# rpng/R-VIO

Measured on AMD Instinct MI355X. Metric: camera frames/sec (KLT+RANSAC track, IMU propagate, MSCKF update, augment/compose), 200 feat / 10-clone window, higher is better.
Workload: dtype f64 (filter) / u8+i32+f32 (KLT); 1 GPU; cfgB: synthetic EuRoC-shaped 752x480 @20Hz, 200 features, 10-clone window, IMU 200 Hz, single stream, equalizer on (CLAHE 3.0, 5x5), corners from the device detector (GFTT + cornerSubPix); parallelism=single GPU

## Files before the change

r-vio_amd/abi.py:

```python
import ctypes as C
import math
import numpy as np

ABI_VERSION = 6

RVIO_PIX_MONO8, RVIO_PIX_RGB8, RVIO_PIX_BGR8, RVIO_PIX_RGBA8, RVIO_PIX_BGRA8 = 0, 1, 2, 3, 4
PIX_CHANNELS = {RVIO_PIX_MONO8: 1, RVIO_PIX_RGB8: 3, RVIO_PIX_BGR8: 3, RVIO_PIX_RGBA8: 4, RVIO_PIX_BGRA8: 4}


class rvio_config(C.Structure):
    _fields_ = [
        ("imu_rate", C.c_double), ("sigma_g", C.c_double), ("sigma_wg", C.c_double),
        ("sigma_a", C.c_double), ("sigma_wa", C.c_double), ("gravity", C.c_double),
        ("small_angle", C.c_double),
        ("width", C.c_int32), ("height", C.c_int32),
        ("fx", C.c_float), ("fy", C.c_float), ("cx", C.c_float), ("cy", C.c_float),
        ("k1", C.c_float), ("k2", C.c_float), ("p1", C.c_float), ("p2", C.c_float), ("k3", C.c_float),
        ("sigma_px", C.c_float), ("sigma_py", C.c_float),
        ("T_bc", C.c_double * 16),
        ("fisheye", C.c_int32),
        ("n_features", C.c_int32), ("max_track_len", C.c_int32), ("min_track_len", C.c_int32),
        ("min_dist", C.c_float), ("qual_lvl", C.c_float),
        ("block_x", C.c_float), ("block_y", C.c_float),
        ("enable_equalizer", C.c_int32), ("use_sampson", C.c_int32),
        ("inlier_thr", C.c_double),
        ("ini_thr_angle", C.c_double), ("ini_thr_displ", C.c_double),
        ("ini_enable_alignment", C.c_int32), ("reserved0", C.c_int32),
    ]


class rvio_imu(C.Structure):
    _fields_ = [("w", C.c_double * 3), ("a", C.c_double * 3), ("t", C.c_double), ("dt", C.c_double)]


IMU_DTYPE = np.dtype([("w", "f8", 3), ("a", "f8", 3), ("t", "f8"), ("dt", "f8")])
assert IMU_DTYPE.itemsize == C.sizeof(rvio_imu) == 64


class rvio_tracks(C.Structure):
    _fields_ = [("n_feat", C.c_int32), ("max_len", C.c_int32),
# ... 188 lines not shown
```

r-vio_amd/csrc/detector.hip:

```cpp
#pragma once

#define DET_NBCAP 64
#define DET_FAST_N 2048
#define DET_FAST_CELLS 4096

struct DetDev {
    const int* first;
    float* eig;
    int* maxkey;
    int* counters;
    int* cell_cnt;
    unsigned long long* cell_ent;
    int* cell_ci;
    int* nb;
    int* nb_cnt;
    int n_cap;
    unsigned long long* prov;
    unsigned long long* cand;
    unsigned long long* acc;
    unsigned char* state;
    float* raw_xy;
    float* xy;
    int* n_out;
    const float* spmask;
    int sp_win;
    int W, H, F;
    float min_dist;
    double quality;
    int max_cells;
};

__device__ __forceinline__ void det_shift(DetDev& d, size_t off) {
    zmove(d.first, off); zmove(d.eig, off); zmove(d.maxkey, off); zmove(d.counters, off); zmove(d.cell_cnt, off); zmove(d.cell_ent, off);
    zmove(d.cell_ci, off); zmove(d.nb, off); zmove(d.nb_cnt, off); zmove(d.prov, off); zmove(d.cand, off); zmove(d.acc, off); zmove(d.state, off);
    zmove(d.raw_xy, off); zmove(d.xy, off); zmove(d.n_out, off);
}
// ... 326 lines not shown
    if (n_list > 0) flush();
}

__device__ __forceinline__ void det_geometry(const DetDev& d, float* md, int* cell, int* gw, int* gh) {
    const float s = (*d.first) ? 1.f : 2.f;
    *md = s * d.min_dist;
    *cell = (int)rintf(*md);
    *gw = (d.W + *cell - 1) / *cell; *gh = (d.H + *cell - 1) / *cell;
}

#define NMS_T 256
__global__ __launch_bounds__(NMS_T) void nms_threshold_kernel(DetDev d, size_t bs) {
    det_shift(d, (size_t)blockIdx.z * bs);
    const int W = d.W;
    const int np = d.counters[3];
    const float mx = ord2f(*d.maxkey);
    const float thr = (float)((double)mx * d.quality);
    float md; int cell, gw, gh;
    det_geometry(d, &md, &cell, &gw, &gh);
    for (int i = blockIdx.x * NMS_T + threadIdx.x; i < np; i += gridDim.x * NMS_T) {
        const unsigned long long key = d.prov[i];
        const float v = __int_as_float((int)(key >> 32));
        if (!(v > thr)) continue;
        const int idx = (int)(key & 0xffffffffull), x = idx % W, y = idx / W;
        const int ci = atomicAdd(&d.counters[0], 1);
        d.cand[ci] = key;
        const int c = (y / cell) * gw + (x / cell);
        const size_t slot = (size_t)c * cell * cell + atomicAdd(&d.cell_cnt[c], 1);
        d.cell_ent[slot] = key;
        d.cell_ci[slot] = ci;
    }
}

#define NEIGH_T 1024
#define NEIGH_BLOCKS 8
#define NEIGH_BLOCKS_WIDE 2
#define NEIGH_LDS (DET_FAST_N * (8 + 4 + 2 + 2 + 2) + (DET_FAST_CELLS + 2) * 4)

__global__ __launch_bounds__(NEIGH_T) void neigh_kernel(DetDev d, size_t bs) {
    det_shift(d, (size_t)blockIdx.z * bs);
    extern __shared__ __align__(16) unsigned char ndyn[];
    __shared__ int s_w[16];
    const int W = d.W, tid = threadIdx.x;
    float md; int cell, gw, gh;
    det_geometry(d, &md, &cell, &gw, &gh);
    const double md2 = (double)md * (double)md;
    const int n = d.counters[0], ncell = gw * gh;
    if (n <= DET_FAST_N && ncell <= DET_FAST_CELLS) {
        unsigned long long* fkey = (unsigned long long*)ndyn;
        unsigned int* fxy = (unsigned int*)(fkey + DET_FAST_N);
        int* cstart = (int*)(fxy + DET_FAST_N);
        unsigned short* fcell = (unsigned short*)(cstart + DET_FAST_CELLS + 2);
        unsigned short* fslot = fcell + DET_FAST_N;
        unsigned short* order = fslot + DET_FAST_N;
        for (int c = tid; c < ncell; c += NEIGH_T) cstart[c] = 0;
        __syncthreads();
        for (int c = tid; c < n; c += NEIGH_T) {
            const unsigned long long key = d.cand[c];
            const int idx = (int)(key & 0xffffffffull), x = idx % W, y = idx / W;
            const int cc = (y / cell) * gw + (x / cell);
            fkey[c] = key; fxy[c] = (unsigned)x | ((unsigned)y << 16); fcell[c] = (unsigned short)cc;
            fslot[c] = (unsigned short)atomicAdd(&cstart[cc], 1);
        }
        __syncthreads();
        {
            const int per = (ncell + NEIGH_T - 1) / NEIGH_T, b0 = tid * per, lane = tid & 63, wv = tid >> 6;
            int sum = 0;
            for (int k = 0; k < per; ++k) if (b0 + k < ncell) sum += cstart[b0 + k];
            const int inc = wave_incl_scan(sum);
            if (lane == 63) s_w[wv] = inc;
            __syncthreads();
            int run = inc - sum;
            for (int w = 0; w < wv; ++w) run += s_w[w];
            for (int k = 0; k < per; ++k) if (b0 + k < ncell) { const int c = cstart[b0 + k]; cstart[b0 + k] = run; run += c; }
            if (tid == NEIGH_T - 1) cstart[ncell] = run;
        }
        __syncthreads();
        for (int c = tid; c < n; c += NEIGH_T) order[cstart[fcell[c]] + fslot[c]] = (unsigned short)c;
        __syncthreads();
        for (int c = blockIdx.x * NEIGH_T + tid; c < n; c += gridDim.x * NEIGH_T) {
            const unsigned long long key = fkey[c];
            const int x = (int)(fxy[c] & 0xffffu), y = (int)(fxy[c] >> 16), xc = x / cell, yc = y / cell;
            const int y1 = yc > 0 ? yc - 1 : 0, y2 = yc + 1 < gh ? yc + 1 : gh - 1, x1 = xc > 0 ? xc - 1 : 0, x2 = xc + 1 < gw ? xc + 1 : gw - 1;
            int m = 0;
            int* list = d.nb + (size_t)c * DET_NBCAP;
            for (int yy = y1; yy <= y2; ++yy) {
                const int e0 = cstart[yy * gw + x1], e1 = cstart[yy * gw + x2 + 1];
                for (int e = e0; e < e1; ++e) {
                    const int j = order[e];
                    if (!(fkey[j] > key)) continue;
                    const float ddx = (float)x - (float)(fxy[j] & 0xffffu), ddy = (float)y - (float)(fxy[j] >> 16);
                    if ((double)(ddx * ddx + ddy * ddy) < md2) { if (m < DET_NBCAP) list[m] = j; ++m; }
                }
            }
            d.nb_cnt[c] = m <= DET_NBCAP ? m : -1;
        }
        return;
    }
    const size_t cap = (size_t)cell * cell;
    for (int c = blockIdx.x * NEIGH_T + tid; c < n && c < d.n_cap; c += gridDim.x * NEIGH_T) {
        const unsigned long long key = d.cand[c];
        const int idx = (int)(key & 0xffffffffull);
        const int x = idx % W, y = idx / W, xc = x / cell, yc = y / cell;
        int cnt9[9], cid9[9];
#pragma unroll
        for (int q = 0; q < 9; ++q) {
            const int xx = xc + (q % 3) - 1, yy = yc + (q / 3) - 1;
            const bool in = xx >= 0 && yy >= 0 && xx < gw && yy < gh;
            cid9[q] = in ? yy * gw + xx : 0;
            cnt9[q] = in ? d.cell_cnt[cid9[q]] : 0;
        }
        int m = 0;
        int* list = d.nb + (size_t)c * DET_NBCAP;
#pragma unroll
        for (int q = 0; q < 9; ++q) {
            const unsigned long long* ent = d.cell_ent + (size_t)cid9[q] * cap;
            const int* eci = d.cell_ci + (size_t)cid9[q] * cap;
            for (int e = 0; e < cnt9[q]; ++e) {
                const unsigned long long k2 = ent[e];
                if (!(k2 > key)) continue;
                const int i2 = (int)(k2 & 0xffffffffull);
                const float ddx = (float)x - (float)(i2 % W), ddy = (float)y - (float)(i2 / W);
                if ((double)(ddx * ddx + ddy * ddy) < md2) { if (m < DET_NBCAP) list[m] = eci[e]; ++m; }
            }
        }
        d.nb_cnt[c] = m <= DET_NBCAP ? m : -1;
    }
}

#define GREEDY_T 1024
#define DET_LDS_ST 32768
__device__ __noinline__ int greedy_general_step(const DetDev& d, int c, int m, unsigned char* lst, int cell, int gw, int gh, double md2) {
    volatile unsigned char* ls = lst;
    volatile unsigned char* gs = d.state;
    const int W = d.W;
    bool drop = false, wait = false;
    auto st_get = [&](int ci) -> unsigned char { return ci < DET_LDS_ST ? ls[ci] : gs[ci]; };
    if (m >= 0) {
        const int* list = d.nb + (size_t)c * DET_NBCAP;
        for (int e = 0; e < m; ++e) { const unsigned char s2 = st_get(list[e]); drop |= (s2 == 2); wait |= (s2 == 1); }
    } else {
        const size_t cap = (size_t)cell * cell;
        const unsigned long long key = d.cand[c];
        const int idx = (int)(key & 0xffffffffull);
        const int x = idx % W, y = idx / W, xc = x / cell, yc = y / cell;
        const int x1 = xc > 0 ? xc - 1 : 0, y1 = yc > 0 ? yc - 1 : 0, x2 = xc + 1 < gw ? xc + 1 : gw - 1, y2 = yc + 1 < gh ? yc + 1 : gh - 1;
        for (int yy = y1; yy <= y2; ++yy)
            for (int xx = x1; xx <= x2; ++xx) {
                const int cc = yy * gw + xx, cnt = d.cell_cnt[cc];
                const unsigned long long* ent = d.cell_ent + (size_t)cc * cap;
                const int* eci = d.cell_ci + (size_t)cc * cap;
                for (int e = 0; e < cnt; ++e) {
                    const unsigned long long k2 = ent[e];
                    if (!(k2 > key)) continue;
                    const int i2 = (int)(k2 & 0xffffffffull);
                    const float ddx = (float)x - (float)(i2 % W), ddy = (float)y - (float)(i2 / W);
                    if ((double)(ddx * ddx + ddy * ddy) < md2) { const unsigned char s2 = st_get(eci[e]); drop |= (s2 == 2); wait |= (s2 == 1); }
                }
            }
    }
    return (drop ? 1 : 0) | (wait ? 2 : 0);
}
#define DET_LDS_TK 4096
#define DET_CL_N 2048
#define DET_CL_CAP 24576
#define GREEDY_LDS (DET_LDS_TK * 8 + DET_LDS_ST + DET_CL_CAP * 2 + (DET_CL_N + 4) * 4)
__global__ __launch_bounds__(GREEDY_T) void greedy_kernel(DetDev d, size_t bs) {
    det_shift(d, (size_t)blockIdx.z * bs);
    extern __shared__ __align__(16) unsigned char gdyn[];
    unsigned long long* tk = (unsigned long long*)gdyn;
    unsigned char* lst = gdyn + DET_LDS_TK * 8;
    unsigned short* clist = (unsigned short*)(lst + DET_LDS_ST);
    int* coff = (int*)(clist + DET_CL_CAP);
    __shared__ int s_w[16];
    __shared__ int s_flag;
    const int W = d.W, tid = threadIdx.x;
    float md; int cell, gw, gh;
    det_geometry(d, &md, &cell, &gw, &gh);
    const double md2 = (double)md * (double)md;
    const int n = d.counters[0];
    volatile unsigned char* ls = lst;
    volatile unsigned char* gs = d.state;
#define ST_GET(ci) ((ci) < DET_LDS_ST ? ls[(ci)] : gs[(ci)])
#define ST_SET(ci, v) do { if ((ci) < DET_LDS_ST) ls[(ci)] = (v); else gs[(ci)] = (v); } while (0)
    DBG_T(56);
    for (int c = tid; c < n; c += GREEDY_T) ST_SET(c, 1);
    bool packed = n <= DET_CL_N && n <= d.n_cap;
    if (tid == 0) s_flag = 0;
    __syncthreads();
    if (packed) {
        const int c0 = 2 * tid, c1 = 2 * tid + 1, lane = tid & 63, wv = tid >> 6;
        const int m0 = c0 < n ? d.nb_cnt[c0] : 0, m1 = c1 < n ? d.nb_cnt[c1] : 0;
        if (m0 < 0 || m1 < 0) s_flag = 1;
        const int sum = (m0 > 0 ? m0 : 0) + (m1 > 0 ? m1 : 0);
        const int inc = wave_incl_scan(sum);
        if (lane == 63) s_w[wv] = inc;
        __syncthreads();
        int base = inc - sum;
        for (int w = 0; w < wv; ++w) base += s_w[w];
        if (tid == GREEDY_T - 1 && base + sum > DET_CL_CAP) s_flag = 1;
        __syncthreads();
        packed = (s_flag == 0);
        if (packed) {
            auto copy_list = [&](int c, int dst, int m) {
                const int4* l4 = (const int4*)(d.nb + (size_t)c * DET_NBCAP);
                for (int q = 0; q < m; q += 16) {
                    const int4 v0 = l4[q / 4], v1 = l4[q / 4 + 1], v2 = l4[q / 4 + 2], v3 = l4[q / 4 + 3];
                    const int v[16] = {v0.x, v0.y, v0.z, v0.w, v1.x, v1.y, v1.z, v1.w, v2.x, v2.y, v2.z, v2.w, v3.x, v3.y, v3.z, v3.w};
#pragma unroll
                    for (int u = 0; u < 16; ++u) if (q + u < m) clist[dst + q + u] = (unsigned short)v[u];
                }
            };
            if (c0 < n) { coff[c0] = base; copy_list(c0, base, m0); }
            if (c1 < n) { coff[c1] = base + m0; copy_list(c1, base + m0, m1); }
            if (c0 == n - 1) coff[n] = base + m0;
            if (c1 == n - 1) coff[n] = base + m0 + m1;
        }
    }
    __threadfence_block();
    __syncthreads();
    DBG_T(57);
    int pending, rounds = 0;
    do {
        pending = 0; ++rounds;
        if (rounds == 1) DBG_T(10);
        for (int c = tid; c < n; c += GREEDY_T) {
            if (ST_GET(c) != 1) continue;
            bool drop = false, wait = false;
            const int m = packed ? -2 : (c < d.n_cap ? d.nb_cnt[c] : -1);
            if (m == -2) {
                const int o = coff[c], o1 = coff[c + 1];
                for (int e = o; e < o1 && !drop; e += 8) {
                    int id8[8];
#pragma unroll
                    for (int u = 0; u < 8; ++u) id8[u] = (int)clist[min(e + u, o1 - 1)];
                    unsigned char s8[8];
#pragma unroll
                    for (int u = 0; u < 8; ++u) s8[u] = lst[id8[u]];
#pragma unroll
                    for (int u = 0; u < 8; ++u) { drop |= (s8[u] == 2); wait |= (s8[u] == 1); }
                }
            } else {
                const int dw = greedy_general_step(d, c, m, lst, cell, gw, gh, md2);
                drop = (dw & 1) != 0; wait = (dw & 2) != 0;
            }
            if (rounds == 1) DBG_T(11);
            if (drop) ST_SET(c, 3);
            else if (!wait) ST_SET(c, 2);
            else pending = 1;
        }
        if (rounds == 1) DBG_T(12);
        __threadfence_block();
        pending = __syncthreads_or(pending);
        if (rounds == 1) DBG_T(13);
        if (rounds == 2) DBG_T(14);
    } while (pending);
    DBG_T(59);
#ifdef RVIO_DBG_CLOCKS
    if (tid == 0) { g_dbg[62] = n; g_dbg[63] = rounds; }
#endif
    if (tid == 0) s_flag = 0;
    __syncthreads();
    const bool small = n <= DET_LDS_TK;
    for (int c = tid; c < n; c += GREEDY_T)
        if (ST_GET(c) == 2) {
            const unsigned long long key = d.cand[c];
            if (small) tk[atomicAdd(&s_flag, 1)] = key;
            else d.acc[atomicAdd(&d.counters[1], 1)] = key;
        }
#undef ST_GET
#undef ST_SET
    __threadfence_block();
    __syncthreads();
    const int na = small ? s_flag : ((volatile int*)d.counters)[1];
    const bool in_lds = small || na <= DET_LDS_TK;
    if (!small && in_lds) for (int a = tid; a < na; a += GREEDY_T) tk[a] = d.acc[a];
    __syncthreads();
    for (int a = tid; a < na; a += GREEDY_T) {
        const unsigned long long key = in_lds ? tk[a] : d.acc[a];
        int r = 0;
        if (in_lds) for (int b = 0; b < na; ++b) r += (tk[b] > key) ? 1 : 0;
        else for (int b = 0; b < na; ++b) r += (d.acc[b] > key) ? 1 : 0;
        if (r < d.F) {
            const int idx = (int)(key & 0xffffffffull);
            d.raw_xy[2 * r] = (float)(idx % W); d.raw_xy[2 * r + 1] = (float)(idx / W);
        }
    }
    DBG_T(60);
    if (tid == 0) {
        *d.n_out = na < d.F ? na : d.F;
        *d.maxkey = (int)0x80000000;
        d.counters[3] = 0;
    }
}

#define SP_WIN 7
#define SP_WW (2 * SP_WIN + 1)
#define SP_PW (SP_WW + 2)
#define SP_MARG 12
#define SP_RS (SP_PW + 1 + 2 * SP_MARG)
#define SP_T 256
#define SP_LS 44
__global__ __launch_bounds__(SP_T) void subpix_kernel(const uint8_t* __restrict__ src, int stride, DetDev d, size_t src_bs, size_t bs, int dbg_tag) {
    DBG_I(blockIdx.x == 0 && blockIdx.z == 0, dbg_tag, 2);
    src = zoff(src, src_bs); det_shift(d, (size_t)blockIdx.z * bs);
    __shared__ unsigned char reg[SP_RS * SP_RS];
    __shared__ double s_part[2][4][5];
    const int p = blockIdx.x, tid = threadIdx.x, lane = tid & 63, wv = tid >> 6;
    const int n = *d.n_out;
    if (p >= n) return;
    const int W = d.W, H = d.H;
    const float tx = d.raw_xy[2 * p], ty = d.raw_xy[2 * p + 1];
    const int rx0 = (int)tx - (SP_PW - 1) / 2 - SP_MARG, ry0 = (int)ty - (SP_PW - 1) / 2 - SP_MARG;
    for (int e = tid; e < SP_RS * SP_RS; e += SP_T) {
        const int j = e / SP_RS, i = e % SP_RS;
        reg[e] = src[(size_t)min(max(ry0 + j, 0), H - 1) * stride + min(max(rx0 + i, 0), W - 1)];
    }
    __syncthreads();
    auto pix = [&](int x, int y) -> float {
        const int i = x - rx0, j = y - ry0;
        if ((unsigned)i < (unsigned)SP_RS && (unsigned)j < (unsigned)SP_RS) return (float)reg[j * SP_RS + i];
// ... 402 lines not shown
```

r-vio_amd/csrc/rvio_hip.hip:

```cpp
#include <hip/hip_runtime.h>
#include <atomic>
#include <chrono>
#include <dlfcn.h>
#include <cmath>
#include <cstdio>
#include <cstdlib>
#include <cstring>
#include <map>
#include <mutex>
#include <string>
#include <vector>

#include "../../include/rvio_hip.h"
#include "rvio_dev.h"
#include "frontend_dev.h"
#include "filter_kernels.hip"
#include "filter_kernels2.hip"
#include "solve6.hip"
#include "solve7.hip"
#include "solve9.hip"
#include "landmarks.hip"
#include "odom.hip"
#pragma clang fp contract(off)
#include "frontend_kernels.hip"
// ... 1102 lines not shown
    const DevCfg& d = h->dc;
    int rc = RVIO_OK;
    for (int k = 0; k < h->plan.n_ic; ++k) if ((rc = detector_alloc_set(h, h->dets[k])) != RVIO_OK) return rc;
    for (int k = h->plan.n_ic; k < rvio_hip::kIC; ++k) h->dets[k] = h->dets[0];
    DALLOC(h, h->det_xy2[0], (size_t)2 * d.F); DALLOC(h, h->det_xy2[1], (size_t)2 * d.F); DALLOC(h, h->det_xy2[2], (size_t)2 * d.F);
    DALLOC(h, h->det_nout, 3);
    float* mask = nullptr;
    const size_t mside = (size_t)std::max(31, 2 * (int)std::floor(.5 * h->cfg.min_dist) + 1);
    DALLOC(h, mask, mside * mside);
    for (DetDev* q : {&h->dets[0], &h->dets[1], &h->dets[2]}) { q->xy = h->det_xy2[0]; q->n_out = h->det_nout; q->spmask = mask; q->sp_win = (int)std::floor(.5 * h->cfg.min_dist); }
    return RVIO_OK;
}
static int detector_init(rvio_hip* h) {
    if (h->det_ready) return RVIO_OK;
    int rc = detector_check(h);
    if (rc != RVIO_OK) return rc;
    if (!h->det_in_slab && (rc = detector_alloc(h)) != RVIO_OK) return rc;
    DetDev& q = h->dets[0];
    const int spw = q.sp_win, spww = 2 * spw + 1;
    std::vector<float> hm((size_t)spww * spww);
    for (int i = 0; i < spww; ++i) {
        const float y = (float)(i - spw) / (float)spw;
        const float vy = std::exp(-y * y);
        for (int j = 0; j < spww; ++j) { const float x = (float)(j - spw) / (float)spw; hm[(size_t)i * spww + j] = (float)(vy * std::exp(-x * x)); }
    }
    HIPCHK(h, hipMemcpyAsync(const_cast<float*>(q.spmask), hm.data(), sizeof(float) * hm.size(), hipMemcpyHostToDevice, h->stream));
    HIPCHK(h, hipStreamSynchronize(h->stream));
    if (spw > 15) HIPCHK(h, lds_attr((const void*)subpix_wide_kernel, (int)subpix_wide_lds(spw)));
    std::vector<int> minkey((size_t)h->batch, (int)0x80000000);
    for (DetDev* qq : {&h->dets[0], &h->dets[1], &h->dets[2]})
        HIPCHK(h, hipMemcpy2DAsync(qq->maxkey, h->slab_bytes ? h->slab_bytes : sizeof(int), minkey.data(), sizeof(int), sizeof(int), (size_t)(h->det_in_slab ? h->batch : 1),
                                   hipMemcpyHostToDevice, h->stream));
    HIPCHK(h, hipStreamSynchronize(h->stream));
    HIPCHK(h, lds_attr((const void*)neigh_kernel, (int)NEIGH_LDS));
    HIPCHK(h, lds_attr((const void*)greedy_kernel, (int)GREEDY_LDS));
    h->det_ready = true;
    return RVIO_OK;
}
static DetDev det_view(const rvio_hip* h) {
    DetDev q = h->dets[h->runahead ? h->ic : 0];
    q.xy = h->det_xy2[h->dslot]; q.n_out = h->det_nout + h->dslot;
    return q;
}
static hipStream_t image_stream_of(const rvio_hip* h, int ic) { return ic == 0 ? h->stream_t : h->stream_c; }
static hipStream_t image_stream(const rvio_hip* h) { return h->runahead ? image_stream_of(h, h->ic) : h->ts; }
static int detect_dev(rvio_hip* h, const uint8_t* img, int stride, size_t src_bs, hipEvent_t first_flag_ready) {
    const DevCfg& d = h->dc;
    const size_t bs = h->slab_bytes;
    const unsigned B = (unsigned)h->batch;
    const DetDev q = det_view(h);
    const hipStream_t ds = image_stream(h);
    h->det_set_last = h->runahead ? h->ic : 0;
    if (h->wide_px) {
        if (h->pyr_signal) { hipLaunchKernelGGL(stage_signal_kernel, dim3(1), dim3(64), 0, ds, h->pyr_signal); h->pyr_signal = nullptr; }
        hipLaunchKernelGGL(mineig_nms_strip_kernel, dim3((d.W + DET_SW - 1) / DET_SW, (d.H + DET_SH - 1) / DET_SH, B), dim3(64), 0, ds, img, stride, q, src_bs, bs);
    } else {
        hipLaunchKernelGGL(mineig_nms_kernel, dim3((d.W + DET_TW - 1) / DET_TW, (d.H + DET_FH - 1) / DET_FH, B), dim3(DET_T), 0, ds, img, stride, q, src_bs, bs, (int)h->frame_no, h->pyr_signal);
        h->pyr_signal = nullptr;
    }
    if (first_flag_ready) HIPCHK(h, hipStreamWaitEvent(ds, first_flag_ready, 0));
    hipLaunchKernelGGL(nms_threshold_kernel, dim3(16, 1, B), dim3(NMS_T), 0, ds, q, bs);
    const unsigned neigh_blocks = h->wide_px ? NEIGH_BLOCKS_WIDE : NEIGH_BLOCKS;
    hipLaunchKernelGGL(neigh_kernel, dim3(neigh_blocks, 1, B), dim3(NEIGH_T), NEIGH_LDS, ds, q, bs);
    hipLaunchKernelGGL(greedy_kernel, dim3(1, 1, B), dim3(GREEDY_T), GREEDY_LDS, ds, q, bs);
    launch_subpix(h, q, img, stride, src_bs, B, (int)h->frame_no, ds);
    HIPCHK(h, hipGetLastError());
    return RVIO_OK;
}

static int pix_channels(int fmt) { return fmt == RVIO_PIX_MONO8 ? 1 : (fmt == RVIO_PIX_RGB8 || fmt == RVIO_PIX_BGR8) ? 3 : 4; }
static void launch_gray(rvio_hip* h, const uint8_t* src, int stride, size_t src_bs, uint8_t* dst, hipStream_t st) {
    const DevCfg& d = h->dc;
    const int bgr = (h->pix_fmt == RVIO_PIX_BGR8 || h->pix_fmt == RVIO_PIX_BGRA8) ? 1 : 0;
    const size_t bs = (size_t)d.W * d.H;
    const dim3 g((d.W + 255) / 256, (d.H + 3) / 4, h->batch), b(256);
    const bool wide = d.W % 4 == 0 && stride % 4 == 0 && ((uintptr_t)src & 3) == 0 && src_bs % 4 == 0;
    if (h->pix_ch == 3) {
        if (wide) hipLaunchKernelGGL(gray_kernel4<3>, g, b, 0, st, src, d.W, d.H, stride, bgr, dst, src_bs, bs);
        else hipLaunchKernelGGL(gray_kernel<3>, g, b, 0, st, src, d.W, d.H, stride, bgr, dst, src_bs, bs);
    } else {
        if (wide) hipLaunchKernelGGL(gray_kernel4<4>, g, b, 0, st, src, d.W, d.H, stride, bgr, dst, src_bs, bs);
        else hipLaunchKernelGGL(gray_kernel<4>, g, b, 0, st, src, d.W, d.H, stride, bgr, dst, src_bs, bs);
    }
}
int rvio_hip_get_image_format(const rvio_hip* h) { return h ? h->pix_fmt : RVIO_ERR_INVALID; }
int rvio_hip_set_image_format(rvio_hip* h, int format) {
    if (!h) return RVIO_ERR_INVALID;
    if (format < RVIO_PIX_MONO8 || format > RVIO_PIX_BGRA8) { h->err = "unknown image format"; return RVIO_ERR_INVALID; }
    if (format != RVIO_PIX_MONO8 && !h->front_end) { h->err = "this batch handle was created without its front end: it takes no image"; return RVIO_ERR_UNSUPPORTED; }
    if (format == h->pix_fmt) return RVIO_OK;
    HIPCHK(h, hipSetDevice(h->device));
    { const int rc = drain_all(h); if (rc != RVIO_OK) return rc; }
    const int ch = pix_channels(format);
    const size_t npx = (size_t)h->dc.W * h->dc.H;
    if (ch > 1 && !h->d_gray[0]) {
        uint8_t* p = nullptr;
        HIPCHK(h, hipMalloc((void**)&p, 4 * npx * (size_t)h->batch));
// ... 532 lines not shown
        HIPCHK(h, hipMemcpyAsync(h->hb_img[b], pp, npx, hipMemcpyHostToDevice, h->stream_t));
        if (nc > 0) HIPCHK(h, hipMemcpyAsync(h->hb_cand[b], pp + pin_cand, sizeof(float) * 2 * nc, hipMemcpyHostToDevice, h->stream_t));
        HIPCHK(h, hipEventRecord(h->evPin[ps], h->stream_t));
    }
    h->last_ra = ra;
    if (paranoid_bits() & PAR_SYNC_COPIES) {
        HIPCHK(h, hipStreamSynchronize(h->stream_d));
        HIPCHK(h, hipStreamSynchronize(h->stream_t));
        if (h->stream_c) HIPCHK(h, hipStreamSynchronize(h->stream_c));
    }
    return frame_dev_impl(h, h->hb_img[b], (int)rowb, h->hb_imu[imu_slot], m, cand_xy ? h->hb_cand[b] : nullptr, nc, true);
}
int rvio_hip_frame_points(rvio_hip* h, const float* tracked_xy, const unsigned char* status, int n_pts,
                          const rvio_imu* imu, int m, const float* cand_xy, int n_cand) {
    int rc = rvio_hip_track_points(h, tracked_xy, status, n_pts, imu, m, cand_xy, n_cand);
    if (rc != RVIO_OK) return rc;
    return frame_tail_dev(h, h->d_imu, m);
}

int rvio_hip_get_frame_info(rvio_hip* h, rvio_frame_info* info) {
    if (!h || !info) return RVIO_ERR_INVALID;
    HIPCHK(h, hipSetDevice(h->device));
    SYNC_FRONT(h);
    FilterMeta m;
    double lit_rank = -1.0;
    HIPCHK(h, hipMemcpyAsync(info, h->d_info, sizeof *info, hipMemcpyDeviceToHost, h->stream));
    HIPCHK(h, hipMemcpyAsync(&m, h->meta, sizeof m, hipMemcpyDeviceToHost, h->stream));
    if (h->last_Ab) HIPCHK(h, hipMemcpyAsync(&lit_rank, h->last_Ab + (size_t)h->dc.ldh * (h->dc.ldh - 1) + 5, sizeof lit_rank, hipMemcpyDeviceToHost, h->stream));
    HIPCHK(h, hipStreamSynchronize(h->stream));
    info->n_clones = h->n_clones_host; info->n_feat_accepted = m.n_good; info->n_rows = m.n_rows; info->updated = m.updated;
    info->reserved[0] = m.err;
    info->reserved[1] = (m.updated && lit_rank >= 0) ? (int)lit_rank : -1;
    info->rank_truncated_at = m.updated ? m.trunc_at : -1;
    if (m.err & 4) { h->err = "a device-side stage counter timed out (filter -> book-keeping): the frame sequence is invalid, re-initialise"; return RVIO_ERR_STATE; }
    return RVIO_OK;
}
int rvio_hip_get_pose(rvio_hip* h, double p[3], double q[4]) {
    if (!h) return RVIO_ERR_INVALID;
    HIPCHK(h, hipSetDevice(h->device));
    double buf[8];
    HIPCHK(h, hipMemcpyAsync(buf, h->d_pose, sizeof buf, hipMemcpyDeviceToHost, h->stream));
    HIPCHK(h, hipStreamSynchronize(h->stream));
    if (p) for (int i = 0; i < 3; ++i) p[i] = buf[i];
    if (q) for (int i = 0; i < 4; ++i) q[i] = buf[3 + i];
    return RVIO_OK;
}
int rvio_hip_get_pose_at(rvio_hip* h, int instance, double p[3], double q[4]) {
    if (!h || instance < 0 || instance >= h->batch) return RVIO_ERR_INVALID;
    HIPCHK(h, hipSetDevice(h->device));
    double buf[8];
    HIPCHK(h, hipMemcpyAsync(buf, (const char*)h->d_pose + (size_t)instance * h->slab_bytes, sizeof buf, hipMemcpyDeviceToHost, h->stream));
    HIPCHK(h, hipStreamSynchronize(h->stream));
    if (p) for (int i = 0; i < 3; ++i) p[i] = buf[i];
    if (q) for (int i = 0; i < 4; ++i) q[i] = buf[3 + i];
    return RVIO_OK;
}

}

extern "C" {
int rvio_hip_get_corners(rvio_hip* h, int32_t* n, float* xy, float* raw_xy, float* eig) {
    if (!h) return RVIO_ERR_INVALID;
    FRONT_END_ONLY(h);
    if (!h->det_ready) { h->err = "the device detector has not run (pass a NULL corner list to track/frame)"; return RVIO_ERR_INVALID; }
    HIPCHK(h, hipSetDevice(h->device));
    SYNC_FRONT(h);
// ... 62 lines not shown
        if (h->batch > 1 || !h->plan.fuse_ok || !h->time_imu || n < 1) return RVIO_ERR_UNSUPPORTED;
        HIPCHK(h, hipMalloc(&bx, sizeof(double) * d.xdmax)); HIPCHK(h, hipMalloc(&bP, sizeof(double) * d.dmax * d.dmax));
        HIPCHK(h, hipMemcpyAsync(bx, h->x[h->cur], sizeof(double) * d.xdmax, hipMemcpyDeviceToDevice, h->stream));
        HIPCHK(h, hipMemcpyAsync(bP, h->P[h->cur], sizeof(double) * d.dmax * d.dmax, hipMemcpyDeviceToDevice, h->stream));
    }
    if (which == 11 && (h->pix_ch < 2 || !h->gray_src)) { h->err = "no colour image has been handed over (rvio_hip_set_image_format)"; return RVIO_ERR_UNSUPPORTED; }
    rvio_odom* odt = nullptr;
    if (which == 12) {
        if (!h->odom_ring) { h->err = "the odometry ring was never enabled (rvio_hip_set_odometry)"; return RVIO_ERR_UNSUPPORTED; }
        HIPCHK(h, hipMalloc((void**)&odt, sizeof(rvio_odom) * h->batch));
    }
    LmOut lmt = {nullptr, nullptr, nullptr, nullptr, 0};
    if (which == 10) {
        if (!h->lm.count) return RVIO_ERR_UNSUPPORTED;
        const int rc = lm_alloc(h, &lmt);
        if (rc != RVIO_OK) return rc;
    }
    const bool pre = h->plan.solve9_nt && (h->plan.solve9_nt <= 6 || h->plan.chol_queue);
    const UpdateForms fw = forms_at(h, n, pre, true), fs = forms_at(h, n, pre, false);
    HIPCHK(h, hipEventCreate(&e0)); HIPCHK(h, hipEventCreate(&e1));
    HIPCHK(h, hipEventRecord(e0, h->stream));
    for (int it = 0; it < iters; ++it) {
        if (which == 12) {
            launch_odom(h, odt, h->odom_seq);
        } else
        if (which == 10) {
            launch_landmarks(h, n, lmt);
        } else
        if (which == 8) {
            launch_feat_prop(h, n, h->time_imu, h->time_m, 0, 1);
        } else if (which == 9) {
            if (h->batch > 1 || !h->det_ready) return RVIO_ERR_UNSUPPORTED;
            const DetDev q = [&] { DetDev v = h->dets[h->det_set_last]; v.xy = h->det_xy2[h->dslot]; v.n_out = h->det_nout + h->dslot; return v; }();
            hipLaunchKernelGGL(greedy_kernel, dim3(1, 1, 1), dim3(GREEDY_T), GREEDY_LDS, h->stream, q, h->slab_bytes);
        } else
        if (which == 0) {
            launch_solve(h, fw, n, h->block);
        } else if (which == 1) {
            if (h->batch > 1) return RVIO_ERR_UNSUPPORTED;
            hipLaunchKernelGGL(klt_kernel3, dim3(d.F), dim3(64), 0, h->stream, h->pyr[h->pyr_cur], h->pyr[(h->pyr_cur + 3) % 4], d.levels, h->t.n_pts, h->t.feats,
                               h->t.tracked, h->t.status, (size_t)0, (const unsigned long long*)nullptr, 0ull, h->meta);
        } else if (which == 2) {
            launch_feat_build(h, n, 0, 1);
        } else if (which == 3) {
            launch_gram(h, fw, n);
        } else if (which == 4 || which == 5) {
            launch_ug_final(h, fs, n, h->block, h->P[h->cur ^ 1], which == 4, which == 5, false);
        } else if (which == 7) {
            launch_ug_final(h, fw, n, h->block, h->P[h->cur ^ 1], true, true, false);
        } else if (which == 6) {
            if (h->batch > 1 || !h->det_ready) return RVIO_ERR_UNSUPPORTED;
            const DetDev q = [&] { DetDev v = h->dets[h->det_set_last]; v.xy = h->det_xy2[h->dslot]; v.n_out = h->det_nout + h->dslot; return v; }();
            const uint8_t* im = h->pyr[h->pyr_cur].img[0];
            launch_subpix(h, q, im, d.W, (size_t)0, 1u, 0, h->stream);
        } else if (which == 11) {
            launch_gray(h, h->gray_src, h->gray_stride, h->gray_bs, h->d_gray[h->gray_slot], h->stream);
        } else return RVIO_ERR_INVALID;
    }
    HIPCHK(h, hipEventRecord(e1, h->stream));
    if (which == 0) { h->chol_ready = false; h->chol_async = false; }
    if (which == 8) {
        HIPCHK(h, hipMemcpyAsync(h->x[h->cur], bx, sizeof(double) * d.xdmax, hipMemcpyDeviceToDevice, h->stream));
        HIPCHK(h, hipMemcpyAsync(h->P[h->cur], bP, sizeof(double) * d.dmax * d.dmax, hipMemcpyDeviceToDevice, h->stream));
        h->chol_ready = false;
    }
    HIPCHK(h, hipEventSynchronize(e1));
    float ms = 0;
// ... 182 lines not shown
```

Measured before the change: 11080 frames/s.

## Fuse neighbor-list build into greedy corner selection with LDS-resident cell grid

Merges the neighbor-list kernel and the greedy non-max selection kernel into one launch. For up to 4096 candidates, a single block bins candidates by grid cell in LDS and runs the greedy rounds directly over the 3x3 neighbouring cells, using 8-lane groups and ballots. This avoids writing and reading per-candidate neighbor lists in global memory and removes one launch. Larger inputs fall back to the old path, now with a last-block handoff, and a no-progress condition now raises an error flag. The cost is more redundant distance tests per round, and the extra blocks in the fast path do nothing.

```diff
diff --git a/r-vio_amd/abi.py b/r-vio_amd/abi.py
--- a/r-vio_amd/abi.py
+++ b/r-vio_amd/abi.py
@@ -6,6 +6,9 @@
 
 RVIO_PIX_MONO8, RVIO_PIX_RGB8, RVIO_PIX_BGR8, RVIO_PIX_RGBA8, RVIO_PIX_BGRA8 = 0, 1, 2, 3, 4
 PIX_CHANNELS = {RVIO_PIX_MONO8: 1, RVIO_PIX_RGB8: 3, RVIO_PIX_BGR8: 3, RVIO_PIX_RGBA8: 4, RVIO_PIX_BGRA8: 4}
+
+SEL_N = 4096
+DET_FAST_CELLS = 4096
 
 
 class rvio_config(C.Structure):
diff --git a/r-vio_amd/csrc/detector.hip b/r-vio_amd/csrc/detector.hip
--- a/r-vio_amd/csrc/detector.hip
+++ b/r-vio_amd/csrc/detector.hip
@@ -1,7 +1,7 @@
 #pragma once
 
 #define DET_NBCAP 64
-#define DET_FAST_N 2048
+#define SEL_N 4096
 #define DET_FAST_CELLS 4096
 
 struct DetDev {
@@ -394,104 +394,27 @@
     }
 }
 
-#define NEIGH_T 1024
-#define NEIGH_BLOCKS 8
+#define SEL_T 1024
+#define SEL_BLOCKS 8
 #define NEIGH_BLOCKS_WIDE 2
-#define NEIGH_LDS (DET_FAST_N * (8 + 4 + 2 + 2 + 2) + (DET_FAST_CELLS + 2) * 4)
-
-__global__ __launch_bounds__(NEIGH_T) void neigh_kernel(DetDev d, size_t bs) {
-    det_shift(d, (size_t)blockIdx.z * bs);
-    extern __shared__ __align__(16) unsigned char ndyn[];
-    __shared__ int s_w[16];
-    const int W = d.W, tid = threadIdx.x;
-    float md; int cell, gw, gh;
-    det_geometry(d, &md, &cell, &gw, &gh);
-    const double md2 = (double)md * (double)md;
-    const int n = d.counters[0], ncell = gw * gh;
-    if (n <= DET_FAST_N && ncell <= DET_FAST_CELLS) {
-        unsigned long long* fkey = (unsigned long long*)ndyn;
-        unsigned int* fxy = (unsigned int*)(fkey + DET_FAST_N);
-        int* cstart = (int*)(fxy + DET_FAST_N);
-        unsigned short* fcell = (unsigned short*)(cstart + DET_FAST_CELLS + 2);
-        unsigned short* fslot = fcell + DET_FAST_N;
-        unsigned short* order = fslot + DET_FAST_N;
-        for (int c = tid; c < ncell; c += NEIGH_T) cstart[c] = 0;
-        __syncthreads();
-        for (int c = tid; c < n; c += NEIGH_T) {
-            const unsigned long long key = d.cand[c];
-            const int idx = (int)(key & 0xffffffffull), x = idx % W, y = idx / W;
-            const int cc = (y / cell) * gw + (x / cell);
-            fkey[c] = key; fxy[c] = (unsigned)x | ((unsigned)y << 16); fcell[c] = (unsigned short)cc;
-            fslot[c] = (unsigned short)atomicAdd(&cstart[cc], 1);
-        }
-        __syncthreads();
-        {
-            const int per = (ncell + NEIGH_T - 1) / NEIGH_T, b0 = tid * per, lane = tid & 63, wv = tid >> 6;
-            int sum = 0;
-            for (int k = 0; k < per; ++k) if (b0 + k < ncell) sum += cstart[b0 + k];
-            const int inc = wave_incl_scan(sum);
-            if (lane == 63) s_w[wv] = inc;
-            __syncthreads();
-            int run = inc - sum;
-            for (int w = 0; w < wv; ++w) run += s_w[w];
-            for (int k = 0; k < per; ++k) if (b0 + k < ncell) { const int c = cstart[b0 + k]; cstart[b0 + k] = run; run += c; }
-            if (tid == NEIGH_T - 1) cstart[ncell] = run;
-        }
-        __syncthreads();
-        for (int c = tid; c < n; c += NEIGH_T) order[cstart[fcell[c]] + fslot[c]] = (unsigned short)c;
-        __syncthreads();
-        for (int c = blockIdx.x * NEIGH_T + tid; c < n; c += gridDim.x * NEIGH_T) {
-            const unsigned long long key = fkey[c];
-            const int x = (int)(fxy[c] & 0xffffu), y = (int)(fxy[c] >> 16), xc = x / cell, yc = y / cell;
-            const int y1 = yc > 0 ? yc - 1 : 0, y2 = yc + 1 < gh ? yc + 1 : gh - 1, x1 = xc > 0 ? xc - 1 : 0, x2 = xc + 1 < gw ? xc + 1 : gw - 1;
-            int m = 0;
-            int* list = d.nb + (size_t)c * DET_NBCAP;
-            for (int yy = y1; yy <= y2; ++yy) {
-                const int e0 = cstart[yy * gw + x1], e1 = cstart[yy * gw + x2 + 1];
-                for (int e = e0; e < e1; ++e) {
-                    const int j = order[e];
-                    if (!(fkey[j] > key)) continue;
-                    const float ddx = (float)x - (float)(fxy[j] & 0xffffu), ddy = (float)y - (float)(fxy[j] >> 16);
-                    if ((double)(ddx * ddx + ddy * ddy) < md2) { if (m < DET_NBCAP) list[m] = j; ++m; }
-                }
-            }
-            d.nb_cnt[c] = m <= DET_NBCAP ? m : -1;
-        }
-        return;
-    }
-    const size_t cap = (size_t)cell * cell;
-    for (int c = blockIdx.x * NEIGH_T + tid; c < n && c < d.n_cap; c += gridDim.x * NEIGH_T) {
-        const unsigned long long key = d.cand[c];
-        const int idx = (int)(key & 0xffffffffull);
-        const int x = idx % W, y = idx / W, xc = x / cell, yc = y / cell;
-        int cnt9[9], cid9[9];
-#pragma unroll
-        for (int q = 0; q < 9; ++q) {
-            const int xx = xc + (q % 3) - 1, yy = yc + (q / 3) - 1;
-            const bool in = xx >= 0 && yy >= 0 && xx < gw && yy < gh;
-            cid9[q] = in ? yy * gw + xx : 0;
-            cnt9[q] = in ? d.cell_cnt[cid9[q]] : 0;
-        }
-        int m = 0;
-        int* list = d.nb + (size_t)c * DET_NBCAP;
-#pragma unroll
-        for (int q = 0; q < 9; ++q) {
-            const unsigned long long* ent = d.cell_ent + (size_t)cid9[q] * cap;
-            const int* eci = d.cell_ci + (size_t)cid9[q] * cap;
-            for (int e = 0; e < cnt9[q]; ++e) {
-                const unsigned long long k2 = ent[e];
-                if (!(k2 > key)) continue;
-                const int i2 = (int)(k2 & 0xffffffffull);
-                const float ddx = (float)x - (float)(i2 % W), ddy = (float)y - (float)(i2 / W);
-                if ((double)(ddx * ddx + ddy * ddy) < md2) { if (m < DET_NBCAP) list[m] = eci[e]; ++m; }
-            }
-        }
-        d.nb_cnt[c] = m <= DET_NBCAP ? m : -1;
-    }
-}
-
-#define GREEDY_T 1024
 #define DET_LDS_ST 32768
+#define DET_LDS_TK 4096
+#define SEL_G 8
+#define SEL_LDS_A (SEL_N * (8 + 8 + 4 + 4 + 1 + 2 + 2) + (DET_FAST_CELLS + 2) * 4)
+#define SEL_LDS_B (DET_LDS_TK * 8 + DET_LDS_ST)
+#define SEL_LDS (SEL_LDS_A > SEL_LDS_B ? SEL_LDS_A : SEL_LDS_B)
+#define SEL_STATIC_MAX 2048
+static_assert(SEL_LDS + SEL_STATIC_MAX <= RVIO_LDS_LIMIT, "greedy_kernel: static + dynamic LDS must fit a CU");
+static_assert(SEL_N % SEL_T == 0 && SEL_N <= DET_LDS_TK && SEL_N <= 65536, "greedy_kernel: SEL_N candidates per thread in registers, taken keys in LDS");
+#ifdef RVIO_DBG_CLOCKS
+#define SEL_STAMP(i) do { if (threadIdx.x == 0) g_dbg[i] = clock64(); } while (0)
+#define SEL_NOTE(i, v) do { if (threadIdx.x == 0) g_dbg[i] = (v); } while (0)
+#else
+#define SEL_STAMP(i) do { } while (0)
+#define SEL_NOTE(i, v) do { } while (0)
+#endif
+#define DET_ERR_SELECT 16
+
 __device__ __noinline__ int greedy_general_step(const DetDev& d, int c, int m, unsigned char* lst, int cell, int gw, int gh, double md2) {
     volatile unsigned char* ls = lst;
     volatile unsigned char* gs = d.state;
@@ -523,17 +446,138 @@
     }
     return (drop ? 1 : 0) | (wait ? 2 : 0);
 }
-#define DET_LDS_TK 4096
-#define DET_CL_N 2048
-#define DET_CL_CAP 24576
-#define GREEDY_LDS (DET_LDS_TK * 8 + DET_LDS_ST + DET_CL_CAP * 2 + (DET_CL_N + 4) * 4)
-__global__ __launch_bounds__(GREEDY_T) void greedy_kernel(DetDev d, size_t bs) {
+
+template <typename T> __device__ __forceinline__ T lds_ld(const T* p) { return __hip_atomic_load(p, __ATOMIC_RELAXED, __HIP_MEMORY_SCOPE_WORKGROUP); }
+template <typename T> __device__ __forceinline__ void lds_st(T* p, T v) { __hip_atomic_store(p, v, __ATOMIC_RELAXED, __HIP_MEMORY_SCOPE_WORKGROUP); }
+
+__device__ __forceinline__ int select_lds(const DetDev& d, unsigned char* dyn, int n, int cell, int gw, int gh, double md2, FilterMeta* meta, int* s_w) {
+    unsigned long long* tk = (unsigned long long*)dyn;
+    unsigned long long* skey = tk + SEL_N;
+    unsigned int* sxy = (unsigned int*)(skey + SEL_N);
+    unsigned int* scxy = sxy + SEL_N;
+    int* cstart = (int*)(scxy + SEL_N);
+    unsigned char* sst = (unsigned char*)(cstart + DET_FAST_CELLS + 2);
+    unsigned short* pend = (unsigned short*)(sst + SEL_N);
+    __shared__ int s_cnt[3];
+    __shared__ int s_na;
+    const int W = d.W, tid = threadIdx.x, ncell = gw * gh;
+    constexpr int PER = SEL_N / SEL_T;
+    SEL_STAMP(56);
+    for (int c = tid; c < ncell; c += SEL_T) cstart[c] = 0;
+    if (tid < 3) s_cnt[tid] = 0;
+    if (tid == 0) s_na = 0;
+    unsigned long long key[PER];
+#pragma unroll
+    for (int k = 0; k < PER; ++k) { const int c = tid + k * SEL_T; key[k] = c < n ? d.cand[c] : 0ull; }
+    __syncthreads();
+    unsigned int xy[PER], cxy[PER];
+    int cc[PER], slot[PER];
+#pragma unroll
+    for (int k = 0; k < PER; ++k) {
+        cc[k] = 0; slot[k] = 0; xy[k] = 0; cxy[k] = 0;
+        if (tid + k * SEL_T < n) {
+            const int idx = (int)(key[k] & 0xffffffffull), x = idx % W, y = idx / W, xc = x / cell, yc = y / cell;
+            xy[k] = (unsigned)x | ((unsigned)y << 16); cxy[k] = (unsigned)xc | ((unsigned)yc << 16);
+            cc[k] = yc * gw + xc;
+            slot[k] = atomicAdd(&cstart[cc[k]], 1);
+        }
+    }
+    __syncthreads();
+    {
+        const int per = (ncell + SEL_T - 1) / SEL_T, b0 = tid * per, lane = tid & 63, wv = tid >> 6;
+        int sum = 0;
+        for (int k = 0; k < per; ++k) if (b0 + k < ncell) sum += cstart[b0 + k];
+        const int inc = wave_incl_scan(sum);
+        if (lane == 63) s_w[wv] = inc;
+        __syncthreads();
+        int run = inc - sum;
+        for (int w = 0; w < wv; ++w) run += s_w[w];
+        for (int k = 0; k < per; ++k) if (b0 + k < ncell) { const int c = cstart[b0 + k]; cstart[b0 + k] = run; run += c; }
+        if (tid == SEL_T - 1) cstart[ncell] = run;
+    }
+    __syncthreads();
+#pragma unroll
+    for (int k = 0; k < PER; ++k)
+        if (tid + k * SEL_T < n) {
+            const int p = cstart[cc[k]] + slot[k];
+            skey[p] = key[k]; sxy[p] = xy[k]; scxy[p] = cxy[k]; lds_st(sst + p, (unsigned char)1);
+        }
+    __syncthreads();
+    SEL_STAMP(57);
+    const int grp = tid / SEL_G, gl = tid % SEL_G, gsh = (tid & 63) / SEL_G * SEL_G;
+    int rounds = 0, m = n;
+    bool stalled = false;
+    while (m > 0) {
+        const unsigned short* cur = pend + (rounds & 1) * SEL_N;
+        unsigned short* nxt = pend + ((rounds + 1) & 1) * SEL_N;
+        int* ncnt = s_cnt + (rounds + 1) % 3;
+        if (tid == 0) lds_st(s_cnt + (rounds + 2) % 3, 0);
+        for (int i0 = 0; i0 < m; i0 += SEL_T / SEL_G) {
+            const int i = i0 + grp;
+            const bool live = i < m;
+            const int p = live ? (rounds == 0 ? i : (int)cur[i]) : 0;
+            bool drop = false, wait = false;
+            if (live) {
+                const unsigned long long kc = skey[p];
+                const unsigned int pxy = sxy[p], pc = scxy[p];
+                const float fx = (float)(pxy & 0xffffu), fy = (float)(pxy >> 16);
+                const int xc = (int)(pc & 0xffffu), yc = (int)(pc >> 16);
+                const int x1 = xc > 0 ? xc - 1 : 0, x2 = xc + 1 < gw ? xc + 1 : gw - 1;
+                int e0[3], e1[3], span = 0;
+#pragma unroll
+                for (int r = 0; r < 3; ++r) {
+                    const int yy = yc + r - 1, yr = yy < 0 ? 0 : (yy >= gh ? gh - 1 : yy);
+                    const int a = cstart[yr * gw + x1], b = cstart[yr * gw + x2 + 1];
+                    e0[r] = a; e1[r] = yy == yr ? b : a;
+                    span = max(span, e1[r] - e0[r]);
+                }
+                for (int t = gl; t - gl < span; t += 2 * SEL_G) {
+                    unsigned long long kj[6];
+                    unsigned int q[6];
+                    unsigned char sj[6];
+                    bool ok[6];
+#pragma unroll
+                    for (int u = 0; u < 6; ++u) {
+                        const int e = e0[u >> 1] + t + (u & 1) * SEL_G;
+                        ok[u] = e < e1[u >> 1];
+                        const int ee = ok[u] ? e : 0;
+                        kj[u] = skey[ee]; q[u] = sxy[ee]; sj[u] = lds_ld(sst + ee);
+                    }
+#pragma unroll
+                    for (int u = 0; u < 6; ++u) {
+                        if (!ok[u] || !(kj[u] > kc)) continue;
+                        const float ddx = fx - (float)(q[u] & 0xffffu), ddy = fy - (float)(q[u] >> 16);
+                        if ((double)(ddx * ddx + ddy * ddy) < md2) { drop |= (sj[u] == 2); wait |= (sj[u] == 1); }
+                    }
+                }
+            }
+            const unsigned gd = (unsigned)(__builtin_amdgcn_ballot_w64(drop) >> gsh) & ((1u << SEL_G) - 1u);
+            const unsigned gwt = (unsigned)(__builtin_amdgcn_ballot_w64(wait) >> gsh) & ((1u << SEL_G) - 1u);
+            if (live && gl == 0) {
+                if (gd) lds_st(sst + p, (unsigned char)3);
+                else if (!gwt) lds_st(sst + p, (unsigned char)2);
+                else nxt[atomicAdd(ncnt, 1)] = (unsigned short)p;
+            }
+        }
+        __syncthreads();
+        const int m1 = lds_ld(ncnt);
+        ++rounds;
+        if (m1 >= m) { stalled = true; break; }
+        m = m1;
+    }
+    if (stalled && tid == 0 && meta) atomicOr(&meta->err, DET_ERR_SELECT);
+    SEL_STAMP(59);
+    SEL_NOTE(61, 1); SEL_NOTE(62, n); SEL_NOTE(63, rounds);
+    for (int p = tid; p < n; p += SEL_T)
+        if (lds_ld(sst + p) == 2) tk[atomicAdd(&s_na, 1)] = skey[p];
+    __syncthreads();
+    return lds_ld(&s_na);
+}
+
+__global__ __launch_bounds__(SEL_T) void greedy_kernel(DetDev d, size_t bs, FilterMeta* meta) {
     det_shift(d, (size_t)blockIdx.z * bs);
+    if (meta) meta = zoffi(meta, bs, (int)blockIdx.z);
     extern __shared__ __align__(16) unsigned char gdyn[];
-    unsigned long long* tk = (unsigned long long*)gdyn;
-    unsigned char* lst = gdyn + DET_LDS_TK * 8;
-    unsigned short* clist = (unsigned short*)(lst + DET_LDS_ST);
-    int* coff = (int*)(clist + DET_CL_CAP);
     __shared__ int s_w[16];
     __shared__ int s_flag;
     const int W = d.W, tid = threadIdx.x;
@@ -541,104 +585,95 @@
     det_geometry(d, &md, &cell, &gw, &gh);
     const double md2 = (double)md * (double)md;
     const int n = d.counters[0];
-    volatile unsigned char* ls = lst;
-    volatile unsigned char* gs = d.state;
+    unsigned long long* const tk = (unsigned long long*)gdyn;
+    int na;
+    bool in_lds;
+    if (n <= SEL_N && gw * gh <= DET_FAST_CELLS) {
+        if (blockIdx.x != 0) return;
+        na = select_lds(d, gdyn, n, cell, gw, gh, md2, meta, s_w);
+        in_lds = true;
+    } else {
+        {
+            const size_t cap = (size_t)cell * cell;
+            for (int c = blockIdx.x * SEL_T + tid; c < n && c < d.n_cap; c += gridDim.x * SEL_T) {
+                const unsigned long long key = d.cand[c];
+                const int idx = (int)(key & 0xffffffffull);
+                const int x = idx % W, y = idx / W, xc = x / cell, yc = y / cell;
+                int cnt9[9], cid9[9];
+#pragma unroll
+                for (int q = 0; q < 9; ++q) {
+                    const int xx = xc + (q % 3) - 1, yy = yc + (q / 3) - 1;
+                    const bool in = xx >= 0 && yy >= 0 && xx < gw && yy < gh;
+                    cid9[q] = in ? yy * gw + xx : 0;
+                    cnt9[q] = in ? d.cell_cnt[cid9[q]] : 0;
+                }
+                int m = 0;
+                int* list = d.nb + (size_t)c * DET_NBCAP;
+#pragma unroll
+                for (int q = 0; q < 9; ++q) {
+                    const unsigned long long* ent = d.cell_ent + (size_t)cid9[q] * cap;
+                    const int* eci = d.cell_ci + (size_t)cid9[q] * cap;
+                    for (int e = 0; e < cnt9[q]; ++e) {
+                        const unsigned long long k2 = ent[e];
+                        if (!(k2 > key)) continue;
+                        const int i2 = (int)(k2 & 0xffffffffull);
+                        const float ddx = (float)x - (float)(i2 % W), ddy = (float)y - (float)(i2 / W);
+                        if ((double)(ddx * ddx + ddy * ddy) < md2) { if (m < DET_NBCAP) list[m] = eci[e]; ++m; }
+                    }
+                }
+                d.nb_cnt[c] = m <= DET_NBCAP ? m : -1;
+            }
+        }
+        if (!last_block_done(d.counters + 2, (int)gridDim.x)) return;
+        unsigned char* lst = gdyn + DET_LDS_TK * 8;
+        volatile unsigned char* ls = lst;
+        volatile unsigned char* gs = d.state;
 #define ST_GET(ci) ((ci) < DET_LDS_ST ? ls[(ci)] : gs[(ci)])
 #define ST_SET(ci, v) do { if ((ci) < DET_LDS_ST) ls[(ci)] = (v); else gs[(ci)] = (v); } while (0)
-    DBG_T(56);
-    for (int c = tid; c < n; c += GREEDY_T) ST_SET(c, 1);
-    bool packed = n <= DET_CL_N && n <= d.n_cap;
-    if (tid == 0) s_flag = 0;
-    __syncthreads();
-    if (packed) {
-        const int c0 = 2 * tid, c1 = 2 * tid + 1, lane = tid & 63, wv = tid >> 6;
-        const int m0 = c0 < n ? d.nb_cnt[c0] : 0, m1 = c1 < n ? d.nb_cnt[c1] : 0;
-        if (m0 < 0 || m1 < 0) s_flag = 1;
-        const int sum = (m0 > 0 ? m0 : 0) + (m1 > 0 ? m1 : 0);
-        const int inc = wave_incl_scan(sum);
-        if (lane == 63) s_w[wv] = inc;
-        __syncthreads();
-        int base = inc - sum;
-        for (int w = 0; w < wv; ++w) base += s_w[w];
-        if (tid == GREEDY_T - 1 && base + sum > DET_CL_CAP) s_flag = 1;
-        __syncthreads();
-        packed = (s_flag == 0);
-        if (packed) {
-            auto copy_list = [&](int c, int dst, int m) {
-                const int4* l4 = (const int4*)(d.nb + (size_t)c * DET_NBCAP);
-                for (int q = 0; q < m; q += 16) {
-                    const int4 v0 = l4[q / 4], v1 = l4[q / 4 + 1], v2 = l4[q / 4 + 2], v3 = l4[q / 4 + 3];
-                    const int v[16] = {v0.x, v0.y, v0.z, v0.w, v1.x, v1.y, v1.z, v1.w, v2.x, v2.y, v2.z, v2.w, v3.x, v3.y, v3.z, v3.w};
-#pragma unroll
-                    for (int u = 0; u < 16; ++u) if (q + u < m) clist[dst + q + u] = (unsigned short)v[u];
-                }
-            };
-            if (c0 < n) { coff[c0] = base; copy_list(c0, base, m0); }
-            if (c1 < n) { coff[c1] = base + m0; copy_list(c1, base + m0, m1); }
-            if (c0 == n - 1) coff[n] = base + m0;
-            if (c1 == n - 1) coff[n] = base + m0 + m1;
-        }
-    }
-    __threadfence_block();
-    __syncthreads();
-    DBG_T(57);
-    int pending, rounds = 0;
-    do {
-        pending = 0; ++rounds;
-        if (rounds == 1) DBG_T(10);
-        for (int c = tid; c < n; c += GREEDY_T) {
-            if (ST_GET(c) != 1) continue;
-            bool drop = false, wait = false;
-            const int m = packed ? -2 : (c < d.n_cap ? d.nb_cnt[c] : -1);
-            if (m == -2) {
-                const int o = coff[c], o1 = coff[c + 1];
-                for (int e = o; e < o1 && !drop; e += 8) {
-                    int id8[8];
-#pragma unroll
-                    for (int u = 0; u < 8; ++u) id8[u] = (int)clist[min(e + u, o1 - 1)];
-                    unsigned char s8[8];
-#pragma unroll
-                    for (int u = 0; u < 8; ++u) s8[u] = lst[id8[u]];
-#pragma unroll
-                    for (int u = 0; u < 8; ++u) { drop |= (s8[u] == 2); wait |= (s8[u] == 1); }
-                }
-            } else {
-                const int dw = greedy_general_step(d, c, m, lst, cell, gw, gh, md2);
-                drop = (dw & 1) != 0; wait = (dw & 2) != 0;
-            }
-            if (rounds == 1) DBG_T(11);
-            if (drop) ST_SET(c, 3);
-            else if (!wait) ST_SET(c, 2);
-            else pending = 1;
-        }
-        if (rounds == 1) DBG_T(12);
+        SEL_STAMP(56);
+        for (int c = tid; c < n; c += SEL_T) ST_SET(c, 1);
         __threadfence_block();
-        pending = __syncthreads_or(pending);
-        if (rounds == 1) DBG_T(13);
-        if (rounds == 2) DBG_T(14);
-    } while (pending);
-    DBG_T(59);
-#ifdef RVIO_DBG_CLOCKS
-    if (tid == 0) { g_dbg[62] = n; g_dbg[63] = rounds; }
-#endif
-    if (tid == 0) s_flag = 0;
-    __syncthreads();
-    const bool small = n <= DET_LDS_TK;
-    for (int c = tid; c < n; c += GREEDY_T)
-        if (ST_GET(c) == 2) {
-            const unsigned long long key = d.cand[c];
-            if (small) tk[atomicAdd(&s_flag, 1)] = key;
-            else d.acc[atomicAdd(&d.counters[1], 1)] = key;
-        }
+        __syncthreads();
+        SEL_STAMP(57);
+        int pending, progress, rounds = 0;
+        do {
+            pending = 0; progress = 0; ++rounds;
+            for (int c = tid; c < n; c += SEL_T) {
+                if (ST_GET(c) != 1) continue;
+                const int dw = greedy_general_step(d, c, c < d.n_cap ? d.nb_cnt[c] : -1, lst, cell, gw, gh, md2);
+                if (dw & 1) { ST_SET(c, 3); progress = 1; }
+                else if (!(dw & 2)) { ST_SET(c, 2); progress = 1; }
+                else pending = 1;
+            }
+            __threadfence_block();
+            pending = __syncthreads_or(pending);
+            progress = __syncthreads_or(progress);
+            if (pending && (!progress || rounds > n)) {
+                if (tid == 0 && meta) atomicOr(&meta->err, DET_ERR_SELECT);
+                break;
+            }
+        } while (pending);
+        SEL_STAMP(59);
+        SEL_NOTE(61, 2); SEL_NOTE(62, n); SEL_NOTE(63, rounds);
+        if (tid == 0) s_flag = 0;
+        __syncthreads();
+        const bool small = n <= DET_LDS_TK;
+        for (int c = tid; c < n; c += SEL_T)
+            if (ST_GET(c) == 2) {
+                const unsigned long long key = d.cand[c];
+                if (small) tk[atomicAdd(&s_flag, 1)] = key;
+                else d.acc[atomicAdd(&d.counters[1], 1)] = key;
+            }
 #undef ST_GET
 #undef ST_SET
-    __threadfence_block();
-    __syncthreads();
-    const int na = small ? s_flag : ((volatile int*)d.counters)[1];
-    const bool in_lds = small || na <= DET_LDS_TK;
-    if (!small && in_lds) for (int a = tid; a < na; a += GREEDY_T) tk[a] = d.acc[a];
-    __syncthreads();
-    for (int a = tid; a < na; a += GREEDY_T) {
+        __threadfence_block();
+        __syncthreads();
+        na = small ? ((volatile int*)&s_flag)[0] : ((volatile int*)d.counters)[1];
+        in_lds = small || na <= DET_LDS_TK;
+        if (!small && in_lds) for (int a = tid; a < na; a += SEL_T) tk[a] = d.acc[a];
+        __syncthreads();
+    }
+    for (int a = tid; a < na; a += SEL_T) {
         const unsigned long long key = in_lds ? tk[a] : d.acc[a];
         int r = 0;
         if (in_lds) for (int b = 0; b < na; ++b) r += (tk[b] > key) ? 1 : 0;
@@ -648,7 +683,7 @@
             d.raw_xy[2 * r] = (float)(idx % W); d.raw_xy[2 * r + 1] = (float)(idx / W);
         }
     }
-    DBG_T(60);
+    SEL_STAMP(60);
     if (tid == 0) {
         *d.n_out = na < d.F ? na : d.F;
         *d.maxkey = (int)0x80000000;
diff --git a/r-vio_amd/csrc/rvio_hip.hip b/r-vio_amd/csrc/rvio_hip.hip
--- a/r-vio_amd/csrc/rvio_hip.hip
+++ b/r-vio_amd/csrc/rvio_hip.hip
@@ -1158,8 +1158,12 @@
         HIPCHK(h, hipMemcpy2DAsync(qq->maxkey, h->slab_bytes ? h->slab_bytes : sizeof(int), minkey.data(), sizeof(int), sizeof(int), (size_t)(h->det_in_slab ? h->batch : 1),
                                    hipMemcpyHostToDevice, h->stream));
     HIPCHK(h, hipStreamSynchronize(h->stream));
-    HIPCHK(h, lds_attr((const void*)neigh_kernel, (int)NEIGH_LDS));
-    HIPCHK(h, lds_attr((const void*)greedy_kernel, (int)GREEDY_LDS));
+    {
+        hipFuncAttributes fa;
+        HIPCHK(h, hipFuncGetAttributes(&fa, (const void*)greedy_kernel));
+        if (fa.sharedSizeBytes > (size_t)SEL_STATIC_MAX || fa.sharedSizeBytes + (size_t)SEL_LDS > (size_t)RVIO_LDS_LIMIT) { h->err = "greedy_kernel: LDS footprint (static + dynamic) exceeds the 160 KiB of a CU"; return RVIO_ERR_UNSUPPORTED; }
+    }
+    HIPCHK(h, lds_attr((const void*)greedy_kernel, (int)SEL_LDS));
     h->det_ready = true;
     return RVIO_OK;
 }
@@ -1170,6 +1174,9 @@
 }
 static hipStream_t image_stream_of(const rvio_hip* h, int ic) { return ic == 0 ? h->stream_t : h->stream_c; }
 static hipStream_t image_stream(const rvio_hip* h) { return h->runahead ? image_stream_of(h, h->ic) : h->ts; }
+static void launch_select(rvio_hip* h, const DetDev& q, unsigned B, hipStream_t st) {
+    hipLaunchKernelGGL(greedy_kernel, dim3(h->wide_px ? NEIGH_BLOCKS_WIDE : SEL_BLOCKS, 1, B), dim3(SEL_T), SEL_LDS, st, q, h->slab_bytes, h->meta);
+}
 static int detect_dev(rvio_hip* h, const uint8_t* img, int stride, size_t src_bs, hipEvent_t first_flag_ready) {
     const DevCfg& d = h->dc;
     const size_t bs = h->slab_bytes;
@@ -1186,9 +1193,7 @@
     }
     if (first_flag_ready) HIPCHK(h, hipStreamWaitEvent(ds, first_flag_ready, 0));
     hipLaunchKernelGGL(nms_threshold_kernel, dim3(16, 1, B), dim3(NMS_T), 0, ds, q, bs);
-    const unsigned neigh_blocks = h->wide_px ? NEIGH_BLOCKS_WIDE : NEIGH_BLOCKS;
-    hipLaunchKernelGGL(neigh_kernel, dim3(neigh_blocks, 1, B), dim3(NEIGH_T), NEIGH_LDS, ds, q, bs);
-    hipLaunchKernelGGL(greedy_kernel, dim3(1, 1, B), dim3(GREEDY_T), GREEDY_LDS, ds, q, bs);
+    launch_select(h, q, B, ds);
     launch_subpix(h, q, img, stride, src_bs, B, (int)h->frame_no, ds);
     HIPCHK(h, hipGetLastError());
     return RVIO_OK;
@@ -1787,6 +1792,7 @@
     info->reserved[0] = m.err;
     info->reserved[1] = (m.updated && lit_rank >= 0) ? (int)lit_rank : -1;
     info->rank_truncated_at = m.updated ? m.trunc_at : -1;
+    if (m.err & DET_ERR_SELECT) { h->err = "the detector's selection made no progress in a round: its corner list is incomplete"; return RVIO_ERR_STATE; }
     if (m.err & 4) { h->err = "a device-side stage counter timed out (filter -> book-keeping): the frame sequence is invalid, re-initialise"; return RVIO_ERR_STATE; }
     return RVIO_OK;
 }
@@ -1915,7 +1921,7 @@
         } else if (which == 9) {
             if (h->batch > 1 || !h->det_ready) return RVIO_ERR_UNSUPPORTED;
             const DetDev q = [&] { DetDev v = h->dets[h->det_set_last]; v.xy = h->det_xy2[h->dslot]; v.n_out = h->det_nout + h->dslot; return v; }();
-            hipLaunchKernelGGL(greedy_kernel, dim3(1, 1, 1), dim3(GREEDY_T), GREEDY_LDS, h->stream, q, h->slab_bytes);
+            launch_select(h, q, 1u, h->stream);
         } else
         if (which == 0) {
             launch_solve(h, fw, n, h->block);
```

Result: slower. 10400 frames/s (-6.2%).
